# JasonLSC/GSCodec_Studio

Measured on AMD Instinct MI355X. Metric: Msplats/s fwd+bwd @1080p (1M splats), higher is better.
Workload: dtype f32; 1 GPU; BASELINE config 2: load_test_data(scene_grid=3) -> 1006065 gaussians, SH degree 3, 1x1 camera 1920x1080, packed=False, tile 16, fwd + bwd of sum(render); visible=292931, native_step_driver=True, parallelism=camera-sharded dp1

## Files before the change

### gscodec_studio_amd/csrc/rasterize.hip

```cpp
#include "gs_common.h"
#include "rasterize_common.h"
#include "dpp_reduce.h"

#include <cstdlib>
#include <cstring>
#include <type_traits>

#include "rasterize_seg_dev.h"

namespace {

template <int CDIM>
__global__ void __launch_bounds__(GS_WAVE) raster_wave_fwd_kernel(RasterArgs a, uint32_t cnt, uint32_t ch_off) {
    constexpr int REC = 3;
    __shared__ float4 s_rec[(GS_WAVE + 1) * REC];
    const uint32_t lane = threadIdx.x;
    const uint32_t lx = lane & 7u, ly = lane >> 3;
    const uint32_t vitem = xcd_remap(blockIdx.x, gridDim.x, a.xcd_group);
    const TileGeom tg = tile_geom(a, vitem >> 2);
    const uint32_t q = vitem & 3u;
    const float *bg = a.backgrounds ? a.backgrounds + (size_t)tg.cam * a.channels + ch_off : nullptr;

    const LanePixel p = lane_pixel(a, tg, q, lx, ly);
    const float px = p.px, py = p.py;
// ... 6 lines not shown
    float T = 1.f, Tkeep = 1.f, out[CDIM];
    int32_t cur = 0;
    bool done = !p.inside;
#pragma unroll
    for (int k = 0; k < CDIM; ++k) out[k] = 0.f;

    const Rect rect = wave_rect(a, tg, q);
    const int32_t n = rect.empty ? 0 : tg.range_end - tg.range_start;
    const int32_t base0 = tg.range_start & ~(GS_WAVE - 1);
    const int32_t num_batches = n > 0 ? (tg.range_end - base0 + GS_WAVE - 1) / GS_WAVE : 0;
    raise_priority_for(n);
    auto in_range = [&](int32_t idx) { return idx >= tg.range_start && idx < tg.range_end && n > 0; };

    SplatRaw nxt = gather_splat(a, base0 + (int32_t)lane, in_range(base0 + (int32_t)lane));
    const unsigned long long lt_mask = (lane == 0) ? 0ull : (~0ull >> (64 - lane));

    for (int32_t b = 0; b < num_batches; ++b) {
        const int32_t batch_start = base0 + b * GS_WAVE;
        SplatRaw s = nxt;
        CullSplat cs;
        const bool have = in_range(batch_start + (int32_t)lane);
        const bool live = have && cull_prepare(s, cs) && rect_touch(s, cs, rect.x0, rect.x1, rect.y0, rect.y1);
        const unsigned long long lm = __ballot(live);
        const int count = __popcll(lm);
        if (live) {
            const int slot = __popcll(lm & lt_mask);
            write_record<0>(&s_rec[slot * REC], s, nullptr);
            s_rec[slot * REC + 2] = make_float4(0.f, 0.f, __int_as_float(batch_start + (int32_t)lane), __int_as_float(s.g));
        }
        if (b + 1 < num_batches) {
            const int32_t ni = batch_start + GS_WAVE + (int32_t)lane;
            nxt = gather_splat(a, ni, in_range(ni));
        }
        __builtin_amdgcn_wave_barrier();

        auto composite = [&](const float4 &c0, const float4 &c1, const float4 &c2) {
            float col[CDIM];
            const float *cp = a.colors + (size_t)__float_as_int(c2.w) * a.s_color + ch_off;
#pragma unroll
            for (int k = 0; k < CDIM; ++k) col[k] = (uint32_t)k < cnt ? cp[k] : 0.f;
            const int32_t idx = __float_as_int(c2.z);
            const float dx = c0.x - px, dy = c0.y - py;
            SplatSample sm;
            const bool ok = splat_sample(dx, dy, c0.z, c0.w, c1.x, c1.y, sm);
            const float a_eff = ok ? sm.alpha : 0.f;
            const float Tj = T;
            const float next_T = Tj - Tj * a_eff;
            const bool stop = ok && (next_T <= T_MIN);
            const bool use = !done && !stop;
            Tkeep = done ? Tkeep : Tj;
            const float vis = use ? a_eff * Tj : 0.f;
#pragma unroll
            for (int k = 0; k < CDIM; ++k) out[k] += col[k] * vis;
            cur = (use && ok) ? idx : cur;
            done = done || stop;
            T = next_T;
        };
        {
            int j = 0;
            for (; j + 1 < count; j += 2) {
                const float4 a0 = s_rec[j * REC + 0], a1 = s_rec[j * REC + 1], a2 = s_rec[j * REC + 2];
                const float4 b0 = s_rec[j * REC + 3], b1 = s_rec[j * REC + 4], b2 = s_rec[j * REC + 5];
                composite(a0, a1, a2);
                composite(b0, b1, b2);
            }
            if (j < count) {
                const float4 a0 = s_rec[j * REC + 0], a1 = s_rec[j * REC + 1], a2 = s_rec[j * REC + 2];
                composite(a0, a1, a2);
            }
        }
        if (__all(done)) break;
        __builtin_amdgcn_wave_barrier();
    }

    if (p.inside) store_pixel<CDIM>(a, p.pix, a.channels, ch_off, cnt, true, done ? Tkeep : T, out, cur, bg);
}

#ifndef GS_WIDE_FWD_WAVES
#define GS_WIDE_FWD_WAVES 4
#endif
template <int CDIM, bool CKPT>
__global__ void __launch_bounds__(256, CDIM > 9 ? GS_WIDE_FWD_WAVES : 1) raster_tile_fwd_kernel(RasterArgs a, float *__restrict__ ckpt, int32_t seg, int32_t solo_min,
                                                              uint32_t *__restrict__ cost_head, uint32_t *__restrict__ cost_body,
                                                              uint32_t *__restrict__ body_tile, uint32_t *__restrict__ class_count,
                                                              ZeroFill zf, uint32_t ch_off, uint32_t cnt) {
    constexpr bool WIDE = CDIM > 4;
    constexpr int NCW = WIDE ? (CDIM - 2 + 3) / 4 : 0;
    constexpr int REC = WIDE ? 2 + NCW : 3;
    constexpr int BATCH = 256;
    constexpr int NBUF = (WIDE && CDIM > 9) ? 1 : 2;
    static_assert((NBUF * BATCH * REC + REC) * 16 < 65536, "record offsets are 16-bit");
    __shared__ float4 s_rec[NBUF * BATCH * REC + REC];
    constexpr uint32_t NULL_REC_OFF = (uint32_t)NBUF * BATCH * REC * 16u;
    typedef uint16_t list_t;
    __shared__ __attribute__((aligned(16))) list_t s_list[NBUF][4][4][72];
    __shared__ unsigned long long s_mask[NBUF][4][4];
    __shared__ uint32_t s_done[NBUF][4];
    const uint32_t tid = threadIdx.x, lane = tid & 63u;
    const uint32_t w = __builtin_amdgcn_readfirstlane(tid >> 6);
    const uint32_t lx = lane & 7u, ly = lane >> 3;
    if (tid < REC) s_rec[NBUF * BATCH * REC + tid] = make_float4(0.f, tid == 1 ? -__builtin_inff() : 0.f, 0.f, 0.f);
    const bool cost_owner = !WIDE || ch_off == 0u;
    if (CKPT && cost_owner && blockIdx.x == 0 && tid < (uint32_t)COST_CLASSES) class_count[tid] = 0u;
    const TileGeom tg = tile_geom(a, a.tile_order != nullptr ? a.tile_order[blockIdx.x] : xcd_remap(blockIdx.x, gridDim.x, a.xcd_group));
    const uint32_t CH = WIDE ? a.channels : (uint32_t)CDIM, ch0 = WIDE ? ch_off : 0u, nch = WIDE ? cnt : (uint32_t)CDIM;
    const float *bg = a.backgrounds ? a.backgrounds + (size_t)tg.cam * a.channels + ch0 : nullptr;

    const LanePixel p = lane_pixel(a, tg, w, lx, ly);
    const bool inside = p.inside;
    const float px = p.px, py = p.py;

    auto zero_fill_slice = [&]() {
        if (!CKPT || zf.ptr == nullptr) return;
        const size_t base = (size_t)blockIdx.x * zf.per_block;
        for (uint32_t i = tid; i < zf.per_block; i += 256u)
            if (base + i < zf.n) {
                typedef float v4f __attribute__((ext_vector_type(4)));
                __builtin_nontemporal_store((v4f){0.f, 0.f, 0.f, 0.f}, reinterpret_cast<v4f *>(zf.ptr + base + i));
            }
    };

    if (a.masks != nullptr && !a.masks[tg.lin]) {
        if (inside) store_masked_pixel<CDIM>(a.render_colors, p.pix, CH, ch0, nch, bg);
        zero_fill_slice();
        return;
    }

    float qx0[4], qx1[4], qy0[4], qy1[4];
    bool qdone[4];
#pragma unroll
    for (int q = 0; q < 4; ++q) {
        const Rect r = wave_rect(a, tg, (uint32_t)q);
        qx0[q] = r.x0; qx1[q] = r.x1; qy0[q] = r.y0; qy1[q] = r.y1;
        qdone[q] = r.empty;
    }

    float T = 1.f, out[CDIM];
    int32_t cur = 0;
    bool done = !inside;
#pragma unroll
    for (int k = 0; k < CDIM; ++k) out[k] = 0.f;

    const int32_t n = tg.range_end - tg.range_start;
    const int32_t base0 = tg.range_start & ~(GS_WAVE - 1);
    const int32_t num_batches = n > 0 ? (tg.range_end - base0 + BATCH - 1) / BATCH : 0;
    raise_priority_for(n);
    auto in_range = [&](int32_t idx) { return idx >= tg.range_start && idx < tg.range_end; };
    auto load_id = [&](int32_t idx) { return in_range(idx) ? a.flatten_ids[idx] : -1; };
    struct Staged {
        SplatRaw s;
        float col[CDIM];
    };
    auto gather = [&](int32_t g, Staged &o) {
        o.s.g = 0;
        o.s.mx = o.s.my = o.s.ca = o.s.cb = o.s.cc = o.s.opac = 0.f;
#pragma unroll
        for (int k = 0; k < CDIM; ++k) o.col[k] = 0.f;
        if (g >= 0) {
            if constexpr (WIDE) fetch_splat_wide<CDIM>(a, g, o.s, o.col, ch_off, cnt);
            else fetch_splat<CDIM>(a, g, o.s, o.col);
        }
    };
    int32_t id_cur = load_id(base0 + (int32_t)tid);
    int32_t id_nxt = load_id(base0 + BATCH + (int32_t)tid);
    Staged nxt;
    gather(id_cur, nxt);

    CkptCursor ck;
// ... 128 lines not shown
                m = __ballot(touch);
                if (touch) {
                    write_record<CDIM>(&s_rec[slot * REC], st.s, st.col);
                    const uint32_t below = __builtin_amdgcn_mbcnt_hi((uint32_t)(m >> 32), __builtin_amdgcn_mbcnt_lo((uint32_t)m, 0u));
                    s_list[buf][w][w][below] = (list_t)(slot * REC * 16u);
                }
                const uint32_t cnt = (uint32_t)__popcll(m);
                if (lane < 3u && cnt + lane < ((cnt + 3u) & ~3u)) s_list[buf][w][w][cnt + lane] = (list_t)NULL_REC_OFF;
            }
            sid_cur = sid_nxt;
            if (sbi + 1 < n_sb) gather(sid_cur, snx);
            sid_nxt = (sbi + 2 < n_sb) ? load_id(sb_start + 2 * GS_WAVE + (int32_t)lane) : -1;
            __builtin_amdgcn_wave_barrier();
            if (CKPT) ck.before(sb_start, tg.range_end, seg, store_ckpt);
            if (m == 0ull) continue;
            uint32_t cur_off = 0xffffffffu;
            if (CKPT) evals += (uint32_t)__popcll(m);
            walk(&s_list[buf][w][w][0], (uint32_t)__popcll(m), cur_off);
            if (cur_off != 0xffffffffu) cur = sb_start + (int32_t)(record_index<REC>(cur_off >> 4) & 63u);
            if (__all(done)) break;
        }
    } else
    for (int32_t b = 0; b < num_batches; ++b) {
        const uint32_t buf = (uint32_t)b & (uint32_t)(NBUF - 1);
        const int32_t batch_start = base0 + b * BATCH;
        {
            const Staged st = nxt;
            const bool have = id_cur >= 0;
            CullSplat cs;
            const bool live = have && cull_prepare(st.s, cs);
            unsigned long long m[4];
            bool any_touch = false;
#pragma unroll
            for (int q = 0; q < 4; ++q) {
                const bool touch = live && !qdone[q] && rect_touch(st.s, cs, qx0[q], qx1[q], qy0[q], qy1[q]);
                any_touch |= touch;
                m[q] = __ballot(touch);
            }
            if (any_touch) write_record<CDIM>(&s_rec[(buf * BATCH + tid) * REC], st.s, st.col);
            {
                const uint32_t my_off = (buf * BATCH + tid) * REC * 16u;
#pragma unroll
                for (int q = 0; q < 4; ++q) {
                    const uint32_t below = __builtin_amdgcn_mbcnt_hi((uint32_t)(m[q] >> 32), __builtin_amdgcn_mbcnt_lo((uint32_t)m[q], 0u));
                    if ((m[q] >> lane) & 1ull) s_list[buf][w][q][below] = (list_t)my_off;
                    const uint32_t cnt = (uint32_t)__popcll(m[q]);
                    if (lane < 3u && cnt + lane < ((cnt + 3u) & ~3u)) s_list[buf][w][q][cnt + lane] = (list_t)NULL_REC_OFF;
                }
            }
            const bool wave_done = __all(done);
            if (lane == 0) {
#pragma unroll
                for (int q = 0; q < 4; ++q) s_mask[buf][w][q] = m[q];
                s_done[buf][w] = wave_done ? 1u : 0u;
            }
        }
        id_cur = id_nxt;
        if (b + 1 < num_batches) gather(id_cur, nxt);
        id_nxt = (b + 2 < num_batches) ? load_id(batch_start + 2 * BATCH + (int32_t)tid) : -1;
        asm volatile("s_waitcnt lgkmcnt(0)\n\ts_barrier" ::: "memory");
        {
            const uint32_t d0 = s_done[buf][0], d1 = s_done[buf][1], d2 = s_done[buf][2], d3 = s_done[buf][3];
            if (d0 & d1 & d2 & d3) break;
            qdone[0] = qdone[0] || d0; qdone[1] = qdone[1] || d1; qdone[2] = qdone[2] || d2; qdone[3] = qdone[3] || d3;
        }
        uint32_t cur_off = 0xffffffffu;
#pragma unroll 1
        for (int sub = 0; sub < 4; ++sub) {
            const int32_t sb_start = batch_start + sub * GS_WAVE;
            if (sb_start >= tg.range_end) break;
            if (CKPT) ck.before(sb_start, tg.range_end, seg, store_ckpt);
            unsigned long long m = s_mask[buf][sub][w];
            m = ((unsigned long long)(uint32_t)__builtin_amdgcn_readfirstlane((uint32_t)(m >> 32)) << 32) |
                (unsigned long long)(uint32_t)__builtin_amdgcn_readfirstlane((uint32_t)m);
            if (m == 0ull) continue;
            if (CKPT) evals += (uint32_t)__popcll(m);
            walk(&s_list[buf][sub][w][0], (uint32_t)__popcll(m), cur_off);
            if (__all(done)) break;
        }
        if (cur_off != 0xffffffffu) cur = batch_start + (int32_t)record_index<REC>((cur_off >> 4) - buf * (uint32_t)(BATCH * REC));
        if (NBUF == 1) asm volatile("s_waitcnt lgkmcnt(0)\n\ts_barrier" ::: "memory");
    }

    if (CKPT && n > 0) {
        while (ck.next_b < tg.range_end) {
            store_ckpt();
            ck.advance(seg);
        }
        store_cost();
    }
    if (inside) store_pixel<CDIM>(a, p.pix, CH, ch0, nch, cost_owner, T, out, cur, bg);
    zero_fill_slice();
}

constexpr int ORDER_CLASSES = 2048, ORDER_THREADS = 1024, ORDER_PER = 8;
__global__ void __launch_bounds__(ORDER_THREADS) tile_order_kernel(uint32_t n_tiles_all, const int32_t *__restrict__ tile_offsets,
                                                                  uint32_t n_isects, uint32_t *__restrict__ order) {
    __shared__ uint32_t s_cnt[ORDER_CLASSES];
    __shared__ uint32_t s_wave[ORDER_THREADS / 64];
    const uint32_t tid = threadIdx.x;
    s_cnt[tid] = 0u;
    s_cnt[tid + ORDER_THREADS] = 0u;
    auto cls_of = [&](uint32_t t) {
        const uint32_t end = (t + 1u == n_tiles_all) ? n_isects : (uint32_t)tile_offsets[t + 1u];
        const uint32_t len = end - (uint32_t)tile_offsets[t];
        return (uint32_t)(ORDER_CLASSES - 1) - min(len >> 2, (uint32_t)(ORDER_CLASSES - 1));
    };
    uint32_t cls[ORDER_PER];
#pragma unroll
    for (int k = 0; k < ORDER_PER; ++k) {
        const uint32_t t = (uint32_t)k * ORDER_THREADS + tid;
        cls[k] = t < n_tiles_all ? cls_of(t) : 0xffffffffu;
    }
    __syncthreads();
#pragma unroll
    for (int k = 0; k < ORDER_PER; ++k)
        if (cls[k] != 0xffffffffu) atomicAdd(&s_cnt[cls[k]], 1u);
    for (uint32_t t = ORDER_PER * ORDER_THREADS + tid; t < n_tiles_all; t += ORDER_THREADS) atomicAdd(&s_cnt[cls_of(t)], 1u);
    __syncthreads();
    const uint32_t c0 = s_cnt[2u * tid], c1 = s_cnt[2u * tid + 1u];
    uint32_t v = c0 + c1;
#pragma unroll
    for (int off = 1; off < 64; off <<= 1) {
        const uint32_t u = __shfl_up(v, off, 64);
        if ((int)(tid & 63u) >= off) v += u;
    }
    if ((tid & 63u) == 63u) s_wave[tid >> 6] = v;
    __syncthreads();
    const uint32_t wv = (tid & 63u) < (uint32_t)(ORDER_THREADS / 64) ? s_wave[tid & 63u] : 0u;
    uint32_t ws = wv;
#pragma unroll
    for (int off = 1; off < ORDER_THREADS / 64; off <<= 1) {
        const uint32_t u = __shfl_up(ws, off, 64);
        if ((int)(tid & 63u) >= off) ws += u;
    }
    const uint32_t base = __shfl(ws - wv, tid >> 6, 64);
    const uint32_t excl = base + v - (c0 + c1);
    s_cnt[2u * tid] = excl;
    s_cnt[2u * tid + 1u] = excl + c0;
    __syncthreads();
#pragma unroll
    for (int k = 0; k < ORDER_PER; ++k)
        if (cls[k] != 0xffffffffu) order[atomicAdd(&s_cnt[cls[k]], 1u)] = (uint32_t)k * ORDER_THREADS + tid;
    for (uint32_t t = ORDER_PER * ORDER_THREADS + tid; t < n_tiles_all; t += ORDER_THREADS) order[atomicAdd(&s_cnt[cls_of(t)], 1u)] = t;
}

template <int CDIM>
void launch_tile_fwd(const RasterArgs &a, const RasterScratch &v, int32_t solo_min, ZeroFill zf, hipStream_t st, uint32_t ch_off, uint32_t cnt) {
    dim3 grid(a.C * a.tile_width * a.tile_height);
    if (v.ckpt != nullptr)
        hipLaunchKernelGGL((raster_tile_fwd_kernel<CDIM, true>), grid, dim3(256), 0, st, a, v.ckpt, v.seg, solo_min, v.cost_head, v.cost_body, v.body_tile, v.class_count, zf, ch_off, cnt);
    else
        hipLaunchKernelGGL((raster_tile_fwd_kernel<CDIM, false>), grid, dim3(256), 0, st, a, v.ckpt, v.seg, solo_min, v.cost_head, v.cost_body, v.body_tile, v.class_count, zf, ch_off, cnt);
}

template <int CDIM, int CMODE, bool ABS>
__global__ void __launch_bounds__(GS_WAVE) raster_wave_bwd_kernel(RasterArgs a, RasterGradArgs ga, uint32_t cnt, uint32_t ch_off, int use_v_alpha) {
    constexpr int REC = 4;
    constexpr int CR = (CMODE == 2) ? 1 : CDIM;
    __shared__ float4 s_rec[(GS_WAVE + 1) * REC];
    const uint32_t lane = threadIdx.x;
    const uint32_t lx = lane & 7u, ly = lane >> 3;
    const uint32_t vitem = xcd_remap(blockIdx.x, gridDim.x, a.xcd_group);
    const TileGeom tg = tile_geom(a, vitem >> 2);
    if (a.masks != nullptr && !a.masks[tg.lin]) return;
    const uint32_t q = vitem & 3u;
    const Rect rect = wave_rect(a, tg, q);
    if (rect.empty || tg.range_end <= tg.range_start) return;

    const float *bg = a.backgrounds ? a.backgrounds + (size_t)tg.cam * a.channels + ch_off : nullptr;
    const uint32_t ox = lx + 8u * (q & 1u), oy = ly + 8u * (q >> 1);
    const uint32_t x = tg.px0 + ox, y = tg.py0 + oy;
    const bool inside = ox < a.tile_size && oy < a.tile_size && x < a.image_width && y < a.image_height;
    const float px = (float)x + 0.5f, py = (float)y + 0.5f;
    const size_t pix = inside ? ((size_t)tg.cam * a.image_height + y) * a.image_width + x : 0;
    const int64_t vpix = (int64_t)pix * ga.s_vrc_pix + (int64_t)ch_off * ga.s_vrc_ch;
    const float T_final = inside ? 1.f - ga.render_alphas[pix] : 1.f;
    float T = T_final, Bq = 0.f, vc[CR];
    float bg_dot = 0.f;
    if (CMODE != 2) {
#pragma unroll
        for (int k = 0; k < CR; ++k) {
            vc[k] = (inside && (uint32_t)k < cnt) ? ga.v_render_colors[vpix + k * ga.s_vrc_ch] : 0.f;
            if (bg != nullptr && (uint32_t)k < cnt) bg_dot += bg[k] * vc[k];
        }
    } else {
        vc[0] = 0.f;
        if (bg != nullptr && inside)
            for (uint32_t k = 0; k < cnt; ++k) bg_dot += bg[k] * ga.v_render_colors[vpix + k * ga.s_vrc_ch];
    }
    const float v_a = (inside && use_v_alpha) ? ga.v_render_alphas[pix] : 0.f;
    const float Tw = T_final * (v_a - bg_dot);
    const int32_t bin_final = inside ? ga.last_ids[pix] : -1;
    const int32_t bin_max = wave_max_i32(max(-1, bin_final));
    if (bin_max < tg.range_start) return;
    const int32_t first = min(tg.range_end - 1, bin_max);
    const int32_t total = first - tg.range_start + 1;
    const int32_t num_batches = (total + GS_WAVE - 1) / GS_WAVE;
    if (total >= HEAVY_TILE) __builtin_amdgcn_s_setprio(2);

    SplatRaw nxt = gather_splat(a, first - (int32_t)lane, first - (int32_t)lane >= tg.range_start);
    float ncol[CMODE == 0 ? CDIM : 1];
    if (CMODE == 0) {
#pragma unroll
        for (int k = 0; k < CDIM; ++k)
            ncol[k] = (first - (int32_t)lane >= tg.range_start && (uint32_t)k < cnt)
                          ? a.colors[(size_t)nxt.g * a.s_color + ch_off + k] : 0.f;
    }
    const unsigned long long lt_mask = (lane == 0) ? 0ull : (~0ull >> (64 - lane));

    for (int32_t b = 0; b < num_batches; ++b) {
        const int32_t batch_end = first - b * GS_WAVE;
        SplatRaw s = nxt;
        CullSplat cs;
        const int32_t my_idx = batch_end - (int32_t)lane;
        const bool live = (my_idx >= tg.range_start) && cull_prepare(s, cs) && rect_touch(s, cs, rect.x0, rect.x1, rect.y0, rect.y1);
        const unsigned long long lm = __ballot(live);
        const int count = __popcll(lm);
        if (live) {
            const int slot = __popcll(lm & lt_mask);
            float c0 = 0.f, c1 = 0.f, c2 = 0.f, c3 = 0.f;
            if (CMODE == 0) {
                c0 = ncol[0];
                if (CDIM > 1) c1 = ncol[CDIM > 1 ? 1 : 0];
                if (CDIM > 2) c2 = ncol[CDIM > 2 ? 2 : 0];
                if (CDIM > 3) c3 = ncol[CDIM > 3 ? 3 : 0];
            }
            s_rec[slot * REC + 0] = make_float4(s.mx, s.my, -0.5f * LOG2E * s.ca, -LOG2E * s.cb);
            s_rec[slot * REC + 1] = make_float4(-0.5f * LOG2E * s.cc, __log2f(s.opac), c0, c1);
            s_rec[slot * REC + 2] = make_float4(c2, c3, __int_as_float(my_idx), __int_as_float(s.g));
            s_rec[slot * REC + 3] = make_float4(s.ca, s.cb, s.cc, s.opac);
        }
        if (b + 1 < num_batches) {
            const int32_t ni = first - (b + 1) * GS_WAVE - (int32_t)lane;
            nxt = gather_splat(a, ni, ni >= tg.range_start);
            if (CMODE == 0) {
// ... 201 lines not shown
            }
            if (!ROW3 && lane == GS_WAVE - 1) s_acc[t * ACC + 2] = make_float4(C2v, C3v, sm.Ax, sm.Ay);
        };
        {
            Rec ra, rb;
            int ta = next_slot();
            load_rec(ta, ra);
            while (any) {
                any &= ~(1ull << ta);
                const int tb = next_slot();
                load_rec(tb, rb);
                body(ta, ra);
                if (!any) break;
                any &= ~(1ull << tb);
                ta = next_slot();
                load_rec(ta, ra);
                body(tb, rb);
            }
        }
        __builtin_amdgcn_wave_barrier();
        if (ga.packed) {
            if ((touched >> lane) & 1ull) {
                float4 a0 = s_acc[lane * ACC + 0], a1 = s_acc[lane * ACC + 1];
                seg_geom_grads(&s_rec[lane * REC], a0, a1.x, a1.y);
                s_acc[lane * ACC + 0] = a0;
                s_acc[lane * ACC + 1] = a1;
                if (!ABS && CDIM == 3) {
                    const float4 a2 = s_acc[lane * ACC + 2];
                    reinterpret_cast<float *>(&s_acc[lane * ACC + 2])[0] = (a2.x + a2.y) + (a2.z + a2.w);
                }
            }
            __builtin_amdgcn_wave_barrier();
            const uint32_t sub = lane / 12u, comp = lane % 12u;
            const bool comp_on = lane < 60u && (comp < 6u + (uint32_t)CDIM || (ABS && comp >= 10u));
            const float *accf = reinterpret_cast<const float *>(s_acc);
#pragma unroll 1
            for (uint32_t grp = 0; grp < 13u; ++grp) {
                if (((touched >> (grp * 5u)) & 0x1full) == 0ull) continue;
                const uint32_t slot = grp * 5u + sub;
                if (comp_on && slot < 64u && ((touched >> slot) & 1ull)) {
                    const uint32_t g = (uint32_t)__float_as_int(s_rec[slot * REC + 3].z);
                    grad_add<DET ? 1 : 0>(ga, ga.v_means2d + (size_t)g * 16u + comp, (size_t)g, comp, accf[slot * (ACC * 4) + comp]);
                }
            }
        } else if ((touched >> lane) & 1ull) {
            float4 a0 = s_acc[lane * ACC + 0], a1 = s_acc[lane * ACC + 1];
            float4 a2 = s_acc[lane * ACC + 2];
            if (!ABS && CDIM == 3) a2.x = (a2.x + a2.y) + (a2.z + a2.w);
            seg_geom_grads(&s_rec[lane * REC], a0, a1.x, a1.y);
            const size_t g = (size_t)__float_as_int(s_rec[lane * REC + 3].z);
            float *vcol = ga.v_colors + g * CDIM;
            grad_add<DET ? 1 : 0>(ga, vcol, g, 6u, a1.z);
            if (CDIM > 1) grad_add<DET ? 1 : 0>(ga, vcol + 1, g, 7u, a1.w);
            if (CDIM > 2) grad_add<DET ? 1 : 0>(ga, vcol + 2, g, 8u, a2.x);
            if (CDIM > 3) grad_add<DET ? 1 : 0>(ga, vcol + 3, g, 9u, a2.y);
            grad_add<DET ? 1 : 0>(ga, ga.v_means2d + ga.s_xy * g, g, 0u, a0.x);
            grad_add<DET ? 1 : 0>(ga, ga.v_means2d + ga.s_xy * g + 1, g, 1u, a0.y);
            grad_add<DET ? 1 : 0>(ga, ga.v_conics + ga.s_conic * g, g, 2u, a0.z);
            grad_add<DET ? 1 : 0>(ga, ga.v_conics + ga.s_conic * g + 1, g, 3u, a0.w);
            grad_add<DET ? 1 : 0>(ga, ga.v_conics + ga.s_conic * g + 2, g, 4u, a1.x);
            grad_add<DET ? 1 : 0>(ga, ga.v_opacities + ga.s_opac * g, g, 5u, a1.y);
            if (ABS) {
                grad_add<DET ? 1 : 0>(ga, ga.v_means2d_abs + ga.s_abs * g, g, 10u, a2.z);
                grad_add<DET ? 1 : 0>(ga, ga.v_means2d_abs + ga.s_abs * g + 1, g, 11u, a2.w);
            }
        }
        __builtin_amdgcn_wave_barrier();
    }
}

template <int CDIM>
void launch_bwd_seg(const RasterArgs &a, const RasterGradArgs &ga, int use_va, const SegArgs &sg, hipStream_t st) {
    dim3 grid(sg.max_items, 1);
    const bool abs = ga.v_means2d_abs != nullptr, det = ga.det != nullptr;
    if (abs && det) hipLaunchKernelGGL((raster_seg_bwd_kernel<CDIM, true, true>), grid, dim3(GS_WAVE), 0, st, a, ga, use_va, sg);
    else if (abs) hipLaunchKernelGGL((raster_seg_bwd_kernel<CDIM, true, false>), grid, dim3(GS_WAVE), 0, st, a, ga, use_va, sg);
    else if (det) hipLaunchKernelGGL((raster_seg_bwd_kernel<CDIM, false, true>), grid, dim3(GS_WAVE), 0, st, a, ga, use_va, sg);
    else hipLaunchKernelGGL((raster_seg_bwd_kernel<CDIM, false, false>), grid, dim3(GS_WAVE), 0, st, a, ga, use_va, sg);
}

__global__ void __launch_bounds__(GS_BLOCK) seg_items_build_kernel(uint32_t n_tiles_all, uint32_t n_isects, const int32_t *__restrict__ offsets,
                                                                   const uint8_t *__restrict__ masks, int32_t seg, uint32_t n_bounds,
                                                                   const uint32_t *__restrict__ cost_head, const uint32_t *__restrict__ cost_body,
                                                                   const uint32_t *__restrict__ body_tile, uint32_t *__restrict__ class_count,
                                                                   uint2 *__restrict__ items, uint32_t max_items) {
    __shared__ uint32_t s_cnt[COST_CLASSES], s_base[COST_CLASSES];
    if (threadIdx.x < COST_CLASSES) s_cnt[threadIdx.x] = 0;
    __syncthreads();
    const uint32_t u = blockIdx.x * GS_BLOCK + threadIdx.x;
    uint32_t tile = 0, cls = 0, local = 0;
    int32_t k = 0;
    bool valid = false;
    auto range = [&](uint32_t t, int32_t &rs, int32_t &re) {
        rs = offsets[t];
        re = (t + 1 == n_tiles_all) ? (int32_t)n_isects : offsets[t + 1];
    };
    if (u < n_tiles_all) {
        int32_t rs, re;
        range(u, rs, re);
        valid = re > rs && (masks == nullptr || masks[u]);
        tile = u;
        k = rs / seg;
        if (valid) {
            const uint4 c = reinterpret_cast<const uint4 *>(cost_head)[u];
            cls = cost_class(c.x + c.y + c.z + c.w, seg);
        }
    } else if (u - n_tiles_all < n_bounds) {
        k = (int32_t)(u - n_tiles_all);
        const uint32_t t = body_tile[k];
        if (k > 0 && t < n_tiles_all) {
            int32_t rs, re;
            range(t, rs, re);
            valid = (int64_t)rs < (int64_t)k * seg && (int64_t)k * seg < (int64_t)re && (masks == nullptr || masks[t]);
            tile = t;
            if (valid) {
                const uint4 c = reinterpret_cast<const uint4 *>(cost_body)[k];
                cls = cost_class(c.x + c.y + c.z + c.w, seg);
            }
        }
    }
    if (valid) local = atomicAdd(&s_cnt[cls], 1u);
    __syncthreads();
    if (threadIdx.x < COST_CLASSES) {
        const uint32_t c = s_cnt[threadIdx.x];
        s_base[threadIdx.x] = c ? atomicAdd(&class_count[threadIdx.x], c) : 0u;
    }
    __syncthreads();
    if (valid) items[(size_t)cls * max_items + s_base[cls] + local] = make_uint2(tile, (uint32_t)k);
}


__global__ void __launch_bounds__(GS_BLOCK) raster_det_finalize_kernel(uint32_t n_elems, uint32_t channels, const long long *__restrict__ det,
                                                                       RasterGradArgs ga) {
    const uint32_t r = blockIdx.x * GS_BLOCK + threadIdx.x;
    if (r >= n_elems) return;
    const long long *d = det + (size_t)r * 24u;
    auto f = [&](uint32_t c) { return (float)((double)d[c] * GS_DET_INV_LO + (double)d[12u + c] * GS_DET_INV_HI); };
    ga.v_means2d[ga.s_xy * (size_t)r] = f(0);
    ga.v_means2d[ga.s_xy * (size_t)r + 1] = f(1);
    ga.v_conics[ga.s_conic * (size_t)r] = f(2);
    ga.v_conics[ga.s_conic * (size_t)r + 1] = f(3);
    ga.v_conics[ga.s_conic * (size_t)r + 2] = f(4);
    ga.v_opacities[ga.s_opac * (size_t)r] = f(5);
    for (uint32_t k = 0; k < channels; ++k) ga.v_colors[ga.s_color * (size_t)r + k] = f(6u + k);
    if (ga.v_means2d_abs != nullptr) {
        ga.v_means2d_abs[ga.s_abs * (size_t)r] = f(10);
        ga.v_means2d_abs[ga.s_abs * (size_t)r + 1] = f(11);
    }
}

}

namespace {

constexpr uint32_t PLAN_MAGIC = 0x47535033u;

constexpr uint32_t FAST_MAX_CHANNELS = 32;

RasterRoute raster_route_fwd(uint32_t channels, const gs_raster_plan *plan) {
    if (channels <= 4u) return RasterRoute::TILE_NARROW;
    return (channels <= FAST_MAX_CHANNELS && plan != nullptr) ? RasterRoute::TILE_WIDE : RasterRoute::WAVE_GENERIC;
}

bool plan_has_ckpt(const gs_raster_plan &p) { return p.seg > 0 && raster_route_fwd(p.channels, &p) != RasterRoute::WAVE_GENERIC; }

RasterRoute raster_route_bwd(uint32_t channels, const gs_raster_plan *plan, const void *scratch, const float *render_colors,
                             const long long *det, bool absgrad) {
    if (plan == nullptr || scratch == nullptr || !plan_has_ckpt(*plan) || render_colors == nullptr) return RasterRoute::WAVE_GENERIC;
    const RasterRoute fwd = raster_route_fwd(channels, plan);
    if (fwd == RasterRoute::TILE_WIDE && (det != nullptr || (absgrad && raster_wide_chunk(channels) < channels)))
        return RasterRoute::WAVE_GENERIC;
    return fwd;
}

RasterScratch scratch_view(const gs_raster_plan &p, void *scratch) {
    const bool ckpt = plan_has_ckpt(p), tile = raster_route_fwd(p.channels, &p) != RasterRoute::WAVE_GENERIC;
    size_t o = 256;
    auto take = [&](bool on, size_t bytes) -> void * {
        void *r = (on && scratch != nullptr) ? (char *)scratch + o : nullptr;
        if (on) o += (bytes + 255) & ~(size_t)255;
        return r;
    };
    RasterScratch v;
    v.seg = p.seg;
    v.n_bounds = (ckpt ? p.n_isects / (uint32_t)p.seg : 0u) + 2u;
    v.max_items = p.n_tiles_all + v.n_bounds;
    v.class_count = (ckpt && scratch != nullptr) ? (uint32_t *)scratch : nullptr;
    v.items = (uint2 *)take(ckpt, (size_t)COST_CLASSES * v.max_items * sizeof(uint2));
    v.cost_head = (uint32_t *)take(true, (size_t)p.n_tiles_all * 4 * sizeof(uint32_t));
    if (!ckpt) v.cost_head = nullptr;
    v.cost_body = (uint32_t *)take(ckpt, (size_t)v.n_bounds * 4 * sizeof(uint32_t));
    v.body_tile = (uint32_t *)take(ckpt, (size_t)v.n_bounds * sizeof(uint32_t));
    v.ckpt = (float *)take(ckpt, (size_t)v.n_bounds * (p.channels + 1) * 256 * sizeof(float));
    v.tile_order = (uint32_t *)take(tile, (size_t)p.n_tiles_all * sizeof(uint32_t));
    if (p.reserved[0] == 0u || p.n_tiles_all == 0u) v.tile_order = nullptr;
    v.total = o;
    return v;
}

}

int32_t raster_make_plan(uint32_t n_tiles_all, uint32_t n_isects, uint32_t channels, const int32_t *tuning, gs_raster_plan *plan) {
    memset(plan, 0, sizeof(*plan));
    int32_t seg = 256, solo = 2048, xf = 16, xb = 16, order = n_tiles_all <= 24576u;
    if (tuning != nullptr) {
        if (tuning[0] >= 0) seg = ((tuning[0] + 63) / 64) * 64;
        if (tuning[1] >= 0) solo = tuning[1];
        if (tuning[2] >= 0) xf = tuning[2];
        if (tuning[3] >= 0) xb = tuning[3];
        if (tuning[4] >= 0) order = tuning[4] != 0;
    }
    while (seg > 0 && (uint64_t)n_isects / (uint32_t)seg * (channels > 4u ? channels + 1u : 4u) > 65536u * 4u) seg *= 2;
    plan->magic = PLAN_MAGIC;
    plan->n_tiles_all = n_tiles_all;
    plan->n_isects = n_isects;
    plan->channels = channels;
    plan->seg = seg;
    plan->solo_min = solo;
    plan->xcd_fwd = (uint32_t)xf;
    plan->xcd_bwd = (uint32_t)xb;
    plan->reserved[0] = (uint32_t)order;
    plan->scratch_bytes = scratch_view(*plan, nullptr).total;
    return 0;
}

bool raster_plan_ok(const gs_raster_plan *plan, uint32_t n_tiles_all, uint32_t n_isects, uint32_t channels) {
    return plan != nullptr && plan->magic == PLAN_MAGIC && plan->n_tiles_all == n_tiles_all && plan->n_isects == n_isects &&
           plan->channels == channels && plan->seg >= 0 && plan->seg % 64 == 0 &&
           plan->scratch_bytes == scratch_view(*plan, nullptr).total;
}

static gs_raster_plan plan_or_default(const RasterArgs &a, const gs_raster_plan *plan) {
    gs_raster_plan p;
    if (plan == nullptr) raster_make_plan(a.C * a.tile_width * a.tile_height, a.n_isects, a.channels, nullptr, &p);
    return plan != nullptr ? *plan : p;
}

int32_t raster_dispatch_fwd(const RasterArgs &a_in, const gs_raster_plan *plan, void *scratch, void *zero_fill, size_t zero_fill_bytes,
                            hipStream_t st) {
    RasterArgs a = a_in;
    const uint32_t n_tiles_all = a.C * a.tile_width * a.tile_height;
    const gs_raster_plan P = plan_or_default(a, plan);
    const RasterRoute route = raster_route_fwd(a.channels, plan);
    const RasterScratch v = scratch_view(P, scratch);
    ZeroFill zf = {nullptr, 0, 0u};
    if (zero_fill != nullptr && zero_fill_bytes > 0) {
        const size_t n16 = zero_fill_bytes / 16;
        const size_t per = (n16 + n_tiles_all - 1) / (n_tiles_all ? n_tiles_all : 1);
        const bool in_kernel = v.ckpt != nullptr && n_tiles_all > 0 && per <= 16384;
        if (in_kernel) zf = {(float4 *)zero_fill, n16, (uint32_t)per};
        else if (hipMemsetAsync(zero_fill, 0, zero_fill_bytes, st) != hipSuccess) { gs_set_error("rasterize: zero fill failed"); return 1; }
    }
    if (route == RasterRoute::WAVE_GENERIC) {
        a.xcd_group = P.xcd_fwd * 4u;
        for (uint32_t off = 0; off < a.channels; off += 32) {
            uint32_t cnt = min(32u, a.channels - off);
            if (cnt <= 8) launch_fwd<8>(a, cnt, off, st);
            else if (cnt <= 16) launch_fwd<16>(a, cnt, off, st);
            else launch_fwd<32>(a, cnt, off, st);
        }
        return 0;
    }
    a.xcd_group = P.xcd_fwd;
    a.tile_order = v.tile_order;
    if (v.tile_order != nullptr)
        hipLaunchKernelGGL(tile_order_kernel, dim3(1), dim3(ORDER_THREADS), 0, st, n_tiles_all, a.tile_offsets, a.n_isects, v.tile_order);
    const uint32_t chunk = route == RasterRoute::TILE_NARROW ? a.channels : raster_wide_chunk(a.channels);
    for (uint32_t off = 0; off < a.channels; off += chunk) {
        const uint32_t cnt = min(chunk, a.channels - off);
        const ZeroFill z = off == 0u ? zf : ZeroFill{nullptr, 0, 0u};
        switch (route == RasterRoute::TILE_NARROW ? (int)cnt : raster_wide_instance(cnt)) {
            case 1: launch_tile_fwd<1>(a, v, P.solo_min, z, st, off, cnt); break;
            case 2: launch_tile_fwd<2>(a, v, P.solo_min, z, st, off, cnt); break;
            case 3: launch_tile_fwd<3>(a, v, P.solo_min, z, st, off, cnt); break;
            case 4: launch_tile_fwd<4>(a, v, P.solo_min, z, st, off, cnt); break;
            case 8: launch_tile_fwd<8>(a, v, P.solo_min, z, st, off, cnt); break;
            case 9: launch_tile_fwd<9>(a, v, P.solo_min, z, st, off, cnt); break;
            case 12: launch_tile_fwd<12>(a, v, P.solo_min, z, st, off, cnt); break;
            default: launch_tile_fwd<16>(a, v, P.solo_min, z, st, off, cnt); break;
        }
    }
    if (v.ckpt != nullptr)
        hipLaunchKernelGGL(seg_items_build_kernel, dim3(gs_div_up(v.max_items, GS_BLOCK)), dim3(GS_BLOCK), 0, st, n_tiles_all, a.n_isects,
                           a.tile_offsets, a.masks, v.seg, v.n_bounds, v.cost_head, v.cost_body, v.body_tile, v.class_count, v.items, v.max_items);
    return 0;
}

int32_t raster_dispatch_bwd(const RasterArgs &a_in, const RasterGradArgs &ga, const float *render_colors, const gs_raster_plan *plan,
                            void *scratch, hipStream_t st) {
    RasterArgs a = a_in;
    const gs_raster_plan P = plan_or_default(a, plan);
    const int use_va = ga.v_render_alphas != nullptr;
    const uint32_t c = a.channels;
    const RasterRoute route = raster_route_bwd(c, plan, scratch, render_colors, ga.det, ga.v_means2d_abs != nullptr);
    if (route == RasterRoute::WAVE_GENERIC) {
        a.xcd_group = P.xcd_bwd * 4u;
        if (c == 1) launch_bwd<1, 0>(a, ga, 1, 0, use_va, st);
        else if (c == 2) launch_bwd<2, 0>(a, ga, 2, 0, use_va, st);
        else if (c == 3) launch_bwd<3, 0>(a, ga, 3, 0, use_va, st);
        else if (c == 4) launch_bwd<4, 0>(a, ga, 4, 0, use_va, st);
        else if (c <= 8) launch_bwd<8, 1>(a, ga, c, 0, use_va, st);
        else if (c <= 16) launch_bwd<16, 1>(a, ga, c, 0, use_va, st);
        else if (c <= 32) launch_bwd<32, 1>(a, ga, c, 0, use_va, st);
        else launch_bwd<1, 2>(a, ga, c, 0, use_va, st);
    } else {
        const RasterScratch v = scratch_view(P, scratch);
        a.xcd_group = P.xcd_bwd;
        if (route == RasterRoute::TILE_WIDE) {
            raster_seg_bwd_wide(a, ga, use_va, v, render_colors, st);
        } else {
            const SegArgs sg = seg_args(v, render_colors);
            switch (c) {
                case 1: launch_bwd_seg<1>(a, ga, use_va, sg, st); break;
                case 2: launch_bwd_seg<2>(a, ga, use_va, sg, st); break;
                case 3: launch_bwd_seg<3>(a, ga, use_va, sg, st); break;
                default: launch_bwd_seg<4>(a, ga, use_va, sg, st); break;
            }
        }
    }
    if (ga.det != nullptr)
        hipLaunchKernelGGL(raster_det_finalize_kernel, dim3(gs_div_up(a.n_elems, GS_BLOCK)), dim3(GS_BLOCK), 0, st, a.n_elems, c, ga.det, ga);
    return 0;
}
```

### gscodec_studio_amd/csrc/rasterize_common.h

```cpp
#pragma once

#include "gs_common.h"

struct RasterArgs {
    uint32_t C, n_elems, n_isects, channels;
    const float *means2d;
    const float *conics;
    const float *colors;
    const float *opacities;
    const float *backgrounds;
    const uint8_t *masks;
    uint32_t image_width, image_height, tile_size, tile_width, tile_height;
    const int32_t *tile_offsets;
    const int32_t *flatten_ids;
    float *render_colors;
    float *render_alphas;
    int32_t *last_ids;
    uint32_t xcd_group;
    uint32_t s_xy, s_conic, s_color, s_opac;
    uint32_t row16;
    const uint32_t *tile_order;
};

struct ZeroFill {
    float4 *ptr;
    size_t n;
    uint32_t per_block;
};

struct RasterGradArgs {
    const float *render_alphas;
    const int32_t *last_ids;
    const float *v_render_colors;
    const float *v_render_alphas;
    float *v_means2d_abs;
    float *v_means2d;
    float *v_conics;
    float *v_colors;
    float *v_opacities;
    uint32_t s_abs, s_xy, s_conic, s_color, s_opac;
    uint32_t packed;
    int64_t s_vrc_pix, s_vrc_ch;
    long long *det;
};

constexpr float GS_DET_SPLIT = 1024.f;
constexpr float GS_DET_SCALE_LO = 274877906944.f;
constexpr float GS_DET_SCALE_HI = 64.f;
constexpr double GS_DET_INV_LO = 1.0 / 274877906944.0, GS_DET_INV_HI = 1.0 / 64.0;

template <int DET = -1>
GS_DEV void grad_add(const RasterGradArgs &ga, float *p, size_t row, uint32_t comp, float v) {
    if (DET == 1 || (DET < 0 && ga.det != nullptr)) {
        const bool hi = !(fabsf(v) < GS_DET_SPLIT);
        const long long q = __float2ll_rn(v * (hi ? GS_DET_SCALE_HI : GS_DET_SCALE_LO));
        atomicAdd(reinterpret_cast<unsigned long long *>(ga.det + row * 24u + (hi ? 12u : 0u) + comp), (unsigned long long)q);
    } else {
        unsafeAtomicAdd(p, v);
    }
}

GS_DEV float wave_reduce_sum_dpp(float v) {
    v += __int_as_float(__builtin_amdgcn_update_dpp(0, __float_as_int(v), 0x111, 0xf, 0xf, false));
    v += __int_as_float(__builtin_amdgcn_update_dpp(0, __float_as_int(v), 0x112, 0xf, 0xf, false));
    v += __int_as_float(__builtin_amdgcn_update_dpp(0, __float_as_int(v), 0x114, 0xf, 0xf, false));
    v += __int_as_float(__builtin_amdgcn_update_dpp(0, __float_as_int(v), 0x118, 0xf, 0xf, false));
    v += __int_as_float(__builtin_amdgcn_update_dpp(0, __float_as_int(v), 0x142, 0xa, 0xf, false));
    v += __int_as_float(__builtin_amdgcn_update_dpp(0, __float_as_int(v), 0x143, 0xc, 0xf, false));
    return v;
}

enum class RasterRoute { TILE_NARROW, TILE_WIDE, WAVE_GENERIC };

struct RasterScratch {
    uint32_t *class_count;
    uint2 *items;
    uint32_t *cost_head, *cost_body, *body_tile;
    float *ckpt;
    uint32_t *tile_order;
    uint32_t max_items, n_bounds;
    int32_t seg;
    size_t total;
};

inline uint32_t raster_wide_chunk(uint32_t channels) { return channels <= 16u ? channels : (channels + 1u) / 2u; }
inline int raster_wide_instance(uint32_t cnt) { return cnt <= 8u ? 8 : cnt == 9u ? 9 : cnt <= 12u ? 12 : 16; }

int32_t raster_make_plan(uint32_t n_tiles_all, uint32_t n_isects, uint32_t channels, const int32_t *tuning, gs_raster_plan *plan);
bool raster_plan_ok(const gs_raster_plan *plan, uint32_t n_tiles_all, uint32_t n_isects, uint32_t channels);
int32_t raster_dispatch_fwd(const RasterArgs &a, const gs_raster_plan *plan, void *scratch, void *zero_fill, size_t zero_fill_bytes,
                            hipStream_t st);
int32_t raster_dispatch_bwd(const RasterArgs &a, const RasterGradArgs &ga, const float *render_colors, const gs_raster_plan *plan,
                            void *scratch, hipStream_t st);
void raster_seg_bwd_wide(const RasterArgs &a, const RasterGradArgs &ga, int use_va, const RasterScratch &v, const float *render_colors,
                         hipStream_t st);
```

### gscodec_studio_amd/csrc/rasterize_dev.h

```cpp
#pragma once

#include "gs_common.h"
#include "rasterize_common.h"

namespace {

constexpr float LOG2E = 1.4426950408889634f;
constexpr float LN2 = 0.6931471805599453f;
constexpr float ALPHA_MIN = 1.f / 255.f;
constexpr float ALPHA_MAX = 0.999f;
constexpr float T_MIN = 1e-4f;
constexpr float LOG2_255 = 7.994353436858858f;
constexpr int HEAVY_TILE = 1024;
constexpr int COST_CLASSES = 32;
GS_DEV uint32_t cost_class(uint32_t c, int32_t seg) { return min(c * 8u / (uint32_t)seg, (uint32_t)COST_CLASSES - 1u); }

struct SplatSample {
    float pl;
    float araw;
    float alpha;
};
GS_DEV bool splat_sample(float dx, float dy, float qa, float qb, float qc, float lo2, SplatSample &s, bool pre = true) {
    s.pl = __builtin_fmaf(dx, __builtin_fmaf(qb, dy, qa * dx), __builtin_fmaf(qc * dy, dy, lo2));
    s.araw = __builtin_amdgcn_exp2f(s.pl);
// ... 177 lines not shown
    r.x1 = (float)X1 - 0.5f;
    r.y1 = (float)Y1 - 0.5f;
    return r;
}


struct LanePixel {
    bool inside;
    float px, py;
    size_t pix;
};
GS_DEV LanePixel lane_pixel(const RasterArgs &a, const TileGeom &tg, uint32_t q, uint32_t lx, uint32_t ly) {
    const uint32_t ox = lx + 8u * (q & 1u), oy = ly + 8u * (q >> 1);
    const uint32_t x = tg.px0 + ox, y = tg.py0 + oy;
    LanePixel p;
    p.inside = ox < a.tile_size && oy < a.tile_size && x < a.image_width && y < a.image_height;
    p.px = (float)x + 0.5f;
    p.py = (float)y + 0.5f;
    p.pix = ((size_t)tg.cam * a.image_height + y) * a.image_width + x;
    return p;
}

template <int CDIM>
GS_DEV void store_masked_pixel(float *render_colors, size_t pix, uint32_t channels, uint32_t ch_off, uint32_t cnt, const float *bg) {
    if constexpr (CDIM > 0) {
#pragma unroll
        for (int k = 0; k < CDIM; ++k)
            if ((uint32_t)k < cnt) render_colors[pix * channels + ch_off + k] = bg ? bg[k] : 0.f;
    } else {
        for (uint32_t k = 0; k < cnt; ++k) render_colors[pix * channels + ch_off + k] = bg ? bg[k] : 0.f;
    }
}

GS_DEV void raise_priority_for(int32_t n) {
    if (n >= 4 * HEAVY_TILE) __builtin_amdgcn_s_setprio(3);
    else if (n >= 2 * HEAVY_TILE) __builtin_amdgcn_s_setprio(2);
    else if (n >= HEAVY_TILE) __builtin_amdgcn_s_setprio(1);
}

template <int CDIM>
GS_DEV void write_record(float4 *r, const SplatRaw &s, const float *col) {
    auto c = [&](int k) { return k < CDIM ? col[k < CDIM ? k : 0] : 0.f; };
    r[0] = make_float4(s.mx, s.my, -0.5f * LOG2E * s.ca, -LOG2E * s.cb);
    r[1] = make_float4(-0.5f * LOG2E * s.cc, __log2f(s.opac), c(0), c(1));
#pragma unroll
    for (int j = 0; j < (CDIM + 1) / 4; ++j) r[2 + j] = make_float4(c(2 + 4 * j), c(3 + 4 * j), c(4 + 4 * j), c(5 + 4 * j));
}

template <int REC>
GS_DEV uint32_t record_index(uint32_t slot4) {
    return REC == 3 ? (slot4 * 43691u) >> 17 : slot4 / (uint32_t)REC;
}

struct CkptCursor {
    int32_t next_b, next_k;
    GS_DEV void first(bool on, int32_t range_start, int32_t seg) {
        next_b = on ? (range_start / seg + 1) * seg : 0x7fffffff;
        next_k = on ? next_b / seg : 0;
    }
    GS_DEV void advance(int32_t seg) {
        next_b += seg;
        next_k += 1;
    }
    template <class Store>
    GS_DEV void before(int32_t sb_start, int32_t range_end, int32_t seg, Store &&store) {
        if (sb_start == next_b && next_b < range_end) {
            store();
            advance(seg);
        }
    }
};

template <int CDIM>
GS_DEV void store_pixel(const RasterArgs &a, size_t pix, uint32_t channels, uint32_t ch_off, uint32_t cnt, bool owner, float Tf,
                        const float *out, int32_t last_id, const float *bg) {
    if (owner) a.render_alphas[pix] = 1.f - Tf;
#pragma unroll
    for (int k = 0; k < CDIM; ++k)
        if ((uint32_t)k < cnt) a.render_colors[pix * channels + ch_off + k] = bg ? out[k] + Tf * bg[k] : out[k];
    if (owner) a.last_ids[pix] = last_id;
}

struct SegArgs {
    const uint2 *items;
    const uint32_t *class_count;
    uint32_t max_items;
    const float *ckpt;
    const float *render_colors;
    int32_t seg;
};

inline SegArgs seg_args(const RasterScratch &v, const float *render_colors) { return {v.items, v.class_count, v.max_items, v.ckpt, render_colors, v.seg}; }

}
```

### gscodec_studio_amd/csrc/rasterize_seg_dev.h

```cpp
#pragma once

#include "rasterize_dev.h"

namespace {

template <int CDIM>
struct ChanAll {
    static constexpr uint32_t off = 0u, cnt = (uint32_t)CDIM, stride = (uint32_t)CDIM;
};
struct ChanWindow {
    uint32_t off, cnt, stride;
};

GS_DEV bool seg_item(const RasterArgs &a, const SegArgs &sg, TileGeom &tg, int32_t &seg_k, bool &from_ckpt) {
    uint32_t n_work = 0;
#pragma unroll 8
    for (int c = 0; c < COST_CLASSES; ++c) n_work += sg.class_count[c];
    if (blockIdx.x >= n_work) return false;
    uint32_t r = xcd_remap(blockIdx.x, n_work, a.xcd_group);
    int cls = COST_CLASSES - 1;
    for (; cls > 0; --cls) {
        const uint32_t nc = sg.class_count[cls];
        if (r < nc) break;
        r -= nc;
    }
    const uint2 it = sg.items[(size_t)cls * sg.max_items + r];
    seg_k = (int32_t)it.y;
    tg = tile_geom(a, it.x);
    if (a.masks != nullptr && !a.masks[tg.lin]) return false;
    const int32_t tile_end = tg.range_end;
    tg.range_start = max(tg.range_start, seg_k * sg.seg);
    tg.range_end = min(tg.range_end, (seg_k + 1) * sg.seg);
    from_ckpt = tg.range_end < tile_end;
    return true;
}

template <int CDIM, class Chan>
GS_DEV void seg_fetch(const RasterArgs &a, int32_t idx, int32_t range_start, const Chan &ch, SplatRaw &s, float *col) {
    s.g = 0;
    s.mx = s.my = s.ca = s.cb = s.cc = s.opac = 0.f;
#pragma unroll
    for (int k = 0; k < CDIM; ++k) col[k] = 0.f;
    if (idx >= range_start) {
        if constexpr (CDIM > 4) fetch_splat_wide<CDIM>(a, a.flatten_ids[idx], s, col, ch.off, ch.cnt);
        else fetch_splat<CDIM>(a, a.flatten_ids[idx], s, col);
    }
}

template <int CDIM>
struct SegPixels {
    float px0, py0;
    float T[4];
    float Wq[4];
    float vc[4][CDIM];
    int32_t bin_final[4];
    int32_t q_bin_max[4];
    float qx0[4], qy0[4];
    unsigned q_live;
};

template <int CDIM, class Chan>
GS_DEV void seg_pixels_init(const RasterArgs &a, const RasterGradArgs &ga, int use_v_alpha, const SegArgs &sg, const TileGeom &tg,
                            int32_t seg_k, bool from_ckpt, const Chan &ch, uint32_t lane, SegPixels<CDIM> &p) {
    const uint32_t lx = lane & 7u, ly = lane >> 3;
    p.px0 = (float)(tg.px0 + lx) + 0.5f;
    p.py0 = (float)(tg.py0 + ly) + 0.5f;
    p.q_live = 0;
    const float *bg = a.backgrounds ? a.backgrounds + (size_t)tg.cam * a.channels + ch.off : nullptr;
#pragma unroll
    for (int i = 0; i < 4; ++i) {
        const uint32_t ox = lx + 8u * (i & 1), oy = ly + 8u * (i >> 1);
        const uint32_t x = tg.px0 + ox, y = tg.py0 + oy;
        const bool inside = ox < a.tile_size && oy < a.tile_size && x < a.image_width && y < a.image_height;
        const size_t pix = inside ? ((size_t)tg.cam * a.image_height + y) * a.image_width + x : 0;
        const float T_final = inside ? 1.f - ga.render_alphas[pix] : 1.f;
        p.T[i] = T_final;
        float bg_dot = 0.f;
#pragma unroll
        for (int k = 0; k < CDIM; ++k) {
            p.vc[i][k] = (inside && (uint32_t)k < ch.cnt) ? ga.v_render_colors[(int64_t)pix * ga.s_vrc_pix + (int64_t)(ch.off + k) * ga.s_vrc_ch] : 0.f;
            if (bg != nullptr && (uint32_t)k < ch.cnt) bg_dot += bg[k] * p.vc[i][k];
        }
        const float v_a = (inside && use_v_alpha) ? ga.v_render_alphas[pix] : 0.f;
        p.Wq[i] = T_final * (v_a - bg_dot);
        p.bin_final[i] = inside ? ga.last_ids[pix] : -1;
        if (from_ckpt && inside) {
            const float *cb = sg.ckpt + (size_t)(seg_k + 1) * (ch.stride + 1u) * 256 + i * 64 + lane;
            p.T[i] = cb[0];
            float bsum = 0.f;
#pragma unroll
            for (int k = 0; k < CDIM; ++k) {
                if ((uint32_t)k < ch.cnt) {
                    float fin = sg.render_colors[pix * ch.stride + ch.off + k];
                    if (bg != nullptr) fin -= T_final * bg[k];
                    bsum += p.vc[i][k] * (fin - cb[(ch.off + k + 1u) * 256u]);
                }
            }
            p.Wq[i] -= bsum;
        }
        p.q_bin_max[i] = __builtin_amdgcn_readfirstlane(wave_max_i32(p.bin_final[i]));
        if (p.q_bin_max[i] >= tg.range_start) p.q_live |= 1u << i;
        auto sgpr = [](float v) { return __uint_as_float(__builtin_amdgcn_readfirstlane(__float_as_uint(v))); };
        p.qx0[i] = sgpr((float)(tg.px0 + 8u * (i & 1)) + 0.5f);
        p.qy0[i] = sgpr((float)(tg.py0 + 8u * (i >> 1)) + 0.5f);
    }
}

template <int CDIM>
GS_DEV void seg_stage(const SplatRaw &s, const float *col, int32_t batch_end, int32_t range_start, uint32_t lane, const SegPixels<CDIM> &p,
                      unsigned long long (&qm)[4], float4 *rec) {
    CullSplat cs;
    const int32_t my_idx = batch_end - (int32_t)lane;
    const bool live = (my_idx >= range_start) && cull_prepare(s, cs);
    const int32_t batch_lo = max(range_start, batch_end - (GS_WAVE - 1));
#pragma unroll
    for (int i = 0; i < 4; ++i) {
// ... 71 lines not shown
```

Baseline: 1413 Msplats/s.

## Skip backward segments past each tile's last contributing splat

The forward tile kernel now records, per wave, the largest splat index any pixel actually composited (its 'last' index) and writes it to a per-tile buffer. Checkpoints are only written for segment boundaries below that index. The segment item builder drops segments starting beyond the last live splat and stores a clipped end, widening items to uint4. The backward segmented kernel then processes only up to that end, avoiding work on splats hidden after all pixels saturate, at the cost of extra scratch memory and wider item records.

Measured after the change: 1439 Msplats/s, median of 6. 1.9% higher.

```diff
diff --git a/gscodec_studio_amd/csrc/rasterize.hip b/gscodec_studio_amd/csrc/rasterize.hip
--- a/gscodec_studio_amd/csrc/rasterize.hip
+++ b/gscodec_studio_amd/csrc/rasterize.hip
@@ -112,8 +112,8 @@
 template <int CDIM, bool CKPT>
 __global__ void __launch_bounds__(256, CDIM > 9 ? GS_WIDE_FWD_WAVES : 1) raster_tile_fwd_kernel(RasterArgs a, float *__restrict__ ckpt, int32_t seg, int32_t solo_min,
                                                               uint32_t *__restrict__ cost_head, uint32_t *__restrict__ cost_body,
-                                                              uint32_t *__restrict__ body_tile, uint32_t *__restrict__ class_count,
-                                                              ZeroFill zf, uint32_t ch_off, uint32_t cnt) {
+                                                              uint32_t *__restrict__ body_tile, int32_t *__restrict__ tile_last,
+                                                              uint32_t *__restrict__ class_count, ZeroFill zf, uint32_t ch_off, uint32_t cnt) {
     constexpr bool WIDE = CDIM > 4;
     constexpr int NCW = WIDE ? (CDIM - 2 + 3) / 4 : 0;
     constexpr int REC = WIDE ? 2 + NCW : 3;
@@ -408,13 +408,16 @@
         if (NBUF == 1) asm volatile("s_waitcnt lgkmcnt(0)\n\ts_barrier" ::: "memory");
     }
 
+    const int32_t wave_last = __builtin_amdgcn_readfirstlane(wave_max_i32(inside ? cur : -1));
     if (CKPT && n > 0) {
         while (ck.next_b < tg.range_end) {
-            store_ckpt();
+            if (ck.next_b - seg <= wave_last) store_ckpt();
+            else store_cost();
             ck.advance(seg);
         }
         store_cost();
     }
+    if (CKPT && cost_owner && lane == 0) tile_last[tg.lin * 4u + w] = wave_last;
     if (inside) store_pixel<CDIM>(a, p.pix, CH, ch0, nch, cost_owner, T, out, cur, bg);
     zero_fill_slice();
 }
@@ -475,9 +478,9 @@
 void launch_tile_fwd(const RasterArgs &a, const RasterScratch &v, int32_t solo_min, ZeroFill zf, hipStream_t st, uint32_t ch_off, uint32_t cnt) {
     dim3 grid(a.C * a.tile_width * a.tile_height);
     if (v.ckpt != nullptr)
-        hipLaunchKernelGGL((raster_tile_fwd_kernel<CDIM, true>), grid, dim3(256), 0, st, a, v.ckpt, v.seg, solo_min, v.cost_head, v.cost_body, v.body_tile, v.class_count, zf, ch_off, cnt);
+        hipLaunchKernelGGL((raster_tile_fwd_kernel<CDIM, true>), grid, dim3(256), 0, st, a, v.ckpt, v.seg, solo_min, v.cost_head, v.cost_body, v.body_tile, v.tile_last, v.class_count, zf, ch_off, cnt);
     else
-        hipLaunchKernelGGL((raster_tile_fwd_kernel<CDIM, false>), grid, dim3(256), 0, st, a, v.ckpt, v.seg, solo_min, v.cost_head, v.cost_body, v.body_tile, v.class_count, zf, ch_off, cnt);
+        hipLaunchKernelGGL((raster_tile_fwd_kernel<CDIM, false>), grid, dim3(256), 0, st, a, v.ckpt, v.seg, solo_min, v.cost_head, v.cost_body, v.body_tile, v.tile_last, v.class_count, zf, ch_off, cnt);
 }
 
 template <int CDIM, int CMODE, bool ABS>
@@ -845,18 +848,24 @@
 __global__ void __launch_bounds__(GS_BLOCK) seg_items_build_kernel(uint32_t n_tiles_all, uint32_t n_isects, const int32_t *__restrict__ offsets,
                                                                    const uint8_t *__restrict__ masks, int32_t seg, uint32_t n_bounds,
                                                                    const uint32_t *__restrict__ cost_head, const uint32_t *__restrict__ cost_body,
-                                                                   const uint32_t *__restrict__ body_tile, uint32_t *__restrict__ class_count,
-                                                                   uint2 *__restrict__ items, uint32_t max_items) {
+                                                                   const uint32_t *__restrict__ body_tile, const int32_t *__restrict__ tile_last,
+                                                                   uint32_t *__restrict__ class_count, uint4 *__restrict__ items, uint32_t max_items) {
     __shared__ uint32_t s_cnt[COST_CLASSES], s_base[COST_CLASSES];
     if (threadIdx.x < COST_CLASSES) s_cnt[threadIdx.x] = 0;
     __syncthreads();
     const uint32_t u = blockIdx.x * GS_BLOCK + threadIdx.x;
     uint32_t tile = 0, cls = 0, local = 0;
-    int32_t k = 0;
+    int32_t k = 0, end = 0;
     bool valid = false;
     auto range = [&](uint32_t t, int32_t &rs, int32_t &re) {
         rs = offsets[t];
         re = (t + 1 == n_tiles_all) ? (int32_t)n_isects : offsets[t + 1];
+    };
+    auto live = [&](uint32_t t, int32_t start, int32_t re) {
+        const int4 l = reinterpret_cast<const int4 *>(tile_last)[t];
+        const int32_t last = max(max(l.x, l.y), max(l.z, l.w));
+        end = (int32_t)min(min((int64_t)re, ((int64_t)k + 1) * seg), (int64_t)last + 1);
+        return last >= start;
     };
     if (u < n_tiles_all) {
         int32_t rs, re;
@@ -864,6 +873,7 @@
         valid = re > rs && (masks == nullptr || masks[u]);
         tile = u;
         k = rs / seg;
+        valid = valid && live(u, rs, re);
         if (valid) {
             const uint4 c = reinterpret_cast<const uint4 *>(cost_head)[u];
             cls = cost_class(c.x + c.y + c.z + c.w, seg);
@@ -876,6 +886,7 @@
             range(t, rs, re);
             valid = (int64_t)rs < (int64_t)k * seg && (int64_t)k * seg < (int64_t)re && (masks == nullptr || masks[t]);
             tile = t;
+            valid = valid && live(t, k * seg, re);
             if (valid) {
                 const uint4 c = reinterpret_cast<const uint4 *>(cost_body)[k];
                 cls = cost_class(c.x + c.y + c.z + c.w, seg);
@@ -889,7 +900,7 @@
         s_base[threadIdx.x] = c ? atomicAdd(&class_count[threadIdx.x], c) : 0u;
     }
     __syncthreads();
-    if (valid) items[(size_t)cls * max_items + s_base[cls] + local] = make_uint2(tile, (uint32_t)k);
+    if (valid) items[(size_t)cls * max_items + s_base[cls] + local] = make_uint4(tile, (uint32_t)k, (uint32_t)end, 0u);
 }
 
 
@@ -949,11 +960,12 @@
     v.n_bounds = (ckpt ? p.n_isects / (uint32_t)p.seg : 0u) + 2u;
     v.max_items = p.n_tiles_all + v.n_bounds;
     v.class_count = (ckpt && scratch != nullptr) ? (uint32_t *)scratch : nullptr;
-    v.items = (uint2 *)take(ckpt, (size_t)COST_CLASSES * v.max_items * sizeof(uint2));
+    v.items = (uint4 *)take(ckpt, (size_t)COST_CLASSES * v.max_items * sizeof(uint4));
     v.cost_head = (uint32_t *)take(true, (size_t)p.n_tiles_all * 4 * sizeof(uint32_t));
     if (!ckpt) v.cost_head = nullptr;
     v.cost_body = (uint32_t *)take(ckpt, (size_t)v.n_bounds * 4 * sizeof(uint32_t));
     v.body_tile = (uint32_t *)take(ckpt, (size_t)v.n_bounds * sizeof(uint32_t));
+    v.tile_last = (int32_t *)take(ckpt, (size_t)p.n_tiles_all * 4 * sizeof(int32_t));
     v.ckpt = (float *)take(ckpt, (size_t)v.n_bounds * (p.channels + 1) * 256 * sizeof(float));
     v.tile_order = (uint32_t *)take(tile, (size_t)p.n_tiles_all * sizeof(uint32_t));
     if (p.reserved[0] == 0u || p.n_tiles_all == 0u) v.tile_order = nullptr;
@@ -1045,7 +1057,7 @@
     }
     if (v.ckpt != nullptr)
         hipLaunchKernelGGL(seg_items_build_kernel, dim3(gs_div_up(v.max_items, GS_BLOCK)), dim3(GS_BLOCK), 0, st, n_tiles_all, a.n_isects,
-                           a.tile_offsets, a.masks, v.seg, v.n_bounds, v.cost_head, v.cost_body, v.body_tile, v.class_count, v.items, v.max_items);
+                           a.tile_offsets, a.masks, v.seg, v.n_bounds, v.cost_head, v.cost_body, v.body_tile, v.tile_last, v.class_count, v.items, v.max_items);
     return 0;
 }
 
diff --git a/gscodec_studio_amd/csrc/rasterize_common.h b/gscodec_studio_amd/csrc/rasterize_common.h
--- a/gscodec_studio_amd/csrc/rasterize_common.h
+++ b/gscodec_studio_amd/csrc/rasterize_common.h
@@ -74,8 +74,9 @@
 
 struct RasterScratch {
     uint32_t *class_count;
-    uint2 *items;
+    uint4 *items;
     uint32_t *cost_head, *cost_body, *body_tile;
+    int32_t *tile_last;
     float *ckpt;
     uint32_t *tile_order;
     uint32_t max_items, n_bounds;
diff --git a/gscodec_studio_amd/csrc/rasterize_dev.h b/gscodec_studio_amd/csrc/rasterize_dev.h
--- a/gscodec_studio_amd/csrc/rasterize_dev.h
+++ b/gscodec_studio_amd/csrc/rasterize_dev.h
@@ -283,7 +283,7 @@
 }
 
 struct SegArgs {
-    const uint2 *items;
+    const uint4 *items;
     const uint32_t *class_count;
     uint32_t max_items;
     const float *ckpt;
diff --git a/gscodec_studio_amd/csrc/rasterize_seg_dev.h b/gscodec_studio_amd/csrc/rasterize_seg_dev.h
--- a/gscodec_studio_amd/csrc/rasterize_seg_dev.h
+++ b/gscodec_studio_amd/csrc/rasterize_seg_dev.h
@@ -24,14 +24,13 @@
         if (r < nc) break;
         r -= nc;
     }
-    const uint2 it = sg.items[(size_t)cls * sg.max_items + r];
+    const uint4 it = sg.items[(size_t)cls * sg.max_items + r];
     seg_k = (int32_t)it.y;
     tg = tile_geom(a, it.x);
     if (a.masks != nullptr && !a.masks[tg.lin]) return false;
-    const int32_t tile_end = tg.range_end;
+    from_ckpt = (seg_k + 1) * sg.seg < tg.range_end;
     tg.range_start = max(tg.range_start, seg_k * sg.seg);
-    tg.range_end = min(tg.range_end, (seg_k + 1) * sg.seg);
-    from_ckpt = tg.range_end < tile_end;
+    tg.range_end = (int32_t)it.z;
     return true;
 }
 
```
